# tiems90/mosaic

Hardware: AMD Instinct MI355X
Metric: PIP-join points/sec (H3 res 9) at 1/2/4/8 GPUs + achieved HBM GB/s (higher is better)
Workload: dtype f64

## Files before the change

mosaic_amd/csrc/kernels.hip:

```cpp
#include <hip/hip_runtime.h>
#include <stdint.h>

#include <map>
#include <mutex>

#define H3T_QUAL static __constant__ const
#include "h3_core.h"
#include "bng_core.h"
#include "pip_core.h"
#include "h3_ring.h"
#include "kernels.h"
#include "raster.h"

namespace mgpu {

#ifndef MGPU_BLOCK
#define MGPU_BLOCK 64
#endif
constexpr int kBlock = MGPU_BLOCK;
constexpr int kItems = 4;
constexpr int kTile = kBlock * kItems;
constexpr int kStreamBlock = 256;
static_assert(kTile <= 1024, "point-in-tile indices are 10 bits");

// ... 267 lines not shown
  h3::FastHex f = h3::fast_hex2d(lat, lon, res_o, t.k_res > 0 ? t.k_res : h3::k_of_res(res_o), kAllFaces);
  if (f.tie) {
    if (a.tie_host) {
      if (!SLOW) tie_record(a.tie_queue, a.tie_cap, input_pos(a, p), px, py, h3::lattice_key(f.face, f.ijk));
    } else if (!SLOW) {
      *tie = true;
      return Range{0, 0, 0};
    } else {
      route_point(a, p, px, py, &f, tie);
    }
  }
  return probe_range(t, h3::face_ijk_to_h3_fast(f.face, f.ijk, res_o));
}

__device__ __forceinline__ bool chip_is_core(const ChipTableView& t, const Range& r, uint32_t j) {
  return j < 16 ? ((r.core >> j) & 1) : (t.chip_flags[r.first + j] & kChipCore) != 0;
}

template <bool SLOW, int CAND_CAP, int STASH, bool PT_STASH = false>
__device__ __forceinline__ void phase1_item(const ChipTableView& t, int li, const Range& r, double px, double py,
                                            bool& any_tie, uint32_t* s_ncand, uint16_t* s_cand_pj,
                                            double2* s_cand_xy, uint32_t* s_first, uint16_t* s_cnt,
                                            uint32_t* s_mask, uint32_t answer = kNoCellAns, bool deep = false) {
  if (!SLOW && r.count > (uint32_t)kMaskBits) any_tie = true;
  if (deep && r.count == 1 && (r.core & kCoreWhole)) answer = 1u;
  if (answer != kNoCellAns) {
    s_first[li] = r.first;
    if (SLOW) s_cnt[li] = (uint16_t)r.count;
    s_mask[li] = answer;
    return;
  }
  const uint32_t nj = r.count < (uint32_t)kMaskBits ? r.count : (uint32_t)kMaskBits;
  const uint32_t lowm = nj >= 32 ? 0xFFFFFFFFu : ((1u << nj) - 1);
  uint32_t border = ~r.core & lowm;
  for (uint32_t j = 16; j < nj; j++)
    if (t.chip_flags[r.first + j] & kChipCore) border &= ~(1u << j);
  uint32_t mask = lowm & ~border;
  if (border) {
    if (PT_STASH) s_cand_xy[li] = make_double2(px, py);
    const uint32_t nb = __popc(border);
    uint32_t j0 = atomicAdd(s_ncand, nb);
    for (uint32_t b = border; b; b &= b - 1) {
      const uint32_t j = __builtin_ctz(b);
      if (j0 < (uint32_t)CAND_CAP) {
        s_cand_pj[j0] = (uint16_t)(li | (j << 10));
        if (!PT_STASH && j0 < (uint32_t)STASH) s_cand_xy[j0] = make_double2(px, py);
      } else if (!SLOW) {
        any_tie = true;
      } else if (pip::chip_contains_strips(t, r.first + j, px, py)) {
        mask |= 1u << j;
      }
      j0++;
    }
  }
  s_first[li] = r.first;
  if (SLOW) s_cnt[li] = (uint16_t)(r.count > 0xFFFF ? 0xFFFF : r.count);
  s_mask[li] = mask;
}



#ifdef MGPU_STAMPS
#define MGPU_STAMP(ph)                                                              \
  do {                                                                              \
    if (threadIdx.x == 0) {                                                         \
      const uint64_t now = wall_clock64();                                          \
      if ((ph) > 0) atomicAdd(&a.counters[9 + (ph)], (unsigned long long)(now - st_t)); \
      st_t = now;                                                                   \
    }                                                                               \
  } while (0)
#else
#define MGPU_STAMP(ph) \
  do {             \
  } while (0)
#endif

constexpr int kChunk = 4096;
constexpr int kGTile = kTile;
constexpr int kChunkTiles = kChunk / kGTile;
constexpr int kGCandCap = 3 * kTile;
constexpr int kGMixCap = kTile;


template <int IS, bool SLOW, int G = 0>
__device__ __forceinline__ void join_tile(const JoinArgs& a, const uint32_t tile) {
  __shared__ uint32_t s_ncand, s_nmix;
  __shared__ uint32_t s_wave_tot[kBlock / 64];
  __shared__ uint32_t s_first[kTile];
  __shared__ __attribute__((aligned(16))) uint32_t s_mask[kTile];
  __shared__ uint16_t s_cnt[(SLOW || G == 0) ? kTile : 1];
  constexpr int kCap = G ? kGCandCap : kCandCap, kMix = G ? kGMixCap : kMixCap;
  constexpr int kStash = stash_of<G>();
  __shared__ __attribute__((aligned(16))) uint8_t s_buf[G ? kStash * 16 + kCap * 2 + kMix * 2 : kOutCap * 6];
  double2* s_cand_xy = (double2*)s_buf;
  uint16_t* s_cand_pj = (uint16_t*)(s_buf + kStash * 16);
  uint16_t* s_mix = (uint16_t*)(s_buf + kStash * 16 + kCap * 2);
  int32_t* s_out_poly = (int32_t*)s_buf;
  uint16_t* s_out_li = (uint16_t*)(s_buf + kOutCap * 4);
  __shared__ uint16_t s_gidx[G == 2 ? kTile : 1];

  const uint32_t chunk = G ? tile / kChunkTiles : 0u;
  const int64_t gbase = (int64_t)chunk * kChunk;
  const int64_t lbase = gbase + (int64_t)(tile % kChunkTiles) * kGTile;
  uint32_t gcount = 0;
  if (G) {
    const int64_t left = a.n - gbase;
    const uint32_t nm = G == 2 ? a.chunk_mixed[chunk] : (uint32_t)(left <= 0 ? 0 : (left < kChunk ? left : kChunk));
    const uint32_t t0 = (tile % kChunkTiles) * kGTile;
    if (nm <= t0) return;
    gcount = nm - t0 < (uint32_t)kGTile ? nm - t0 : (uint32_t)kGTile;
    if (G == 2)
      for (uint32_t li = threadIdx.x; li < (uint32_t)kTile; li += kBlock)
        s_gidx[li] = li < gcount ? a.mixed_idx[lbase + li] : (uint16_t)0;
  }
  uint32_t ckp[G == 1 ? 4 : 1];
  if (G == 1 && a.in_chunk_pairs) {
    const uint32_t s0 = 4u * threadIdx.x;
    if (s0 + 3 < gcount) {
      const uint4 q = *(const uint4*)(a.pos_of + lbase + s0);
      ckp[0] = q.x, ckp[1] = q.y, ckp[2] = q.z, ckp[3] = q.w;
    } else {
#pragma unroll
      for (int i = 0; i < 4; i++) ckp[i] = s0 + i < gcount ? a.pos_of[lbase + s0 + i] : 0u;
    }
  }
#define MGPU_PT(li) (G == 2 ? gbase + (int64_t)s_gidx[li] : G == 1 ? lbase + (li) : (int64_t)tile * kTile + (li))
#define MGPU_VALID(li) (G ? (uint32_t)(li) < gcount : (int64_t)tile * kTile + (li) < a.n)


#ifdef MGPU_STAMPS
  uint64_t st_t = 0;
#endif
  if (threadIdx.x == 0) {
    s_ncand = 0;
    s_nmix = 0;
  }
  __syncthreads();
  const ChipTableView& t = a.chips;
  const int64_t base = (int64_t)tile * kTile;
  const bool res_match = a.res_match;

  MGPU_STAMP(0);
  bool any_tie = false, any_bad = false;
  uint32_t n_tie_pts = 0;
#ifndef MGPU_NT_POINTS
#define MGPU_NT_POINTS 1
#endif
#if MGPU_NT_POINTS
#define MGPU_LDPT(ptr) __builtin_nontemporal_load(ptr)
#else
#define MGPU_LDPT(ptr) (*(ptr))
#endif
  if (!G && !SLOW && kBlock == 64 && t.raster_mode != kRasterNone && res_match && (IS == MGPU_H3 || a.res == t.res)) {
    const int lane = threadIdx.x;
    double bx[kItems], by[kItems];
#pragma unroll
    for (int k = 0; k < kItems; k++) {
      const int64_t p = base + k * kBlock + lane;
      bx[k] = by[k] = 0.0;
      if (p < a.n) {
        bx[k] = MGPU_LDPT(&a.x[p]);
        by[k] = MGPU_LDPT(&a.y[p]);
      }
    }
    uint32_t ri[kItems], gix[kItems], sb[kItems];
#pragma unroll
    for (int k = 0; k < kItems; k++) {
// ... 53 lines not shown
      if (q < nlist) {
        bool ok, tie;
        uint32_t gi;
        Range r = chip_probe<IS, SLOW>(a, base + li, px, py, &ok, &tie, &gi);
        if (gi != kNoEntry) r = grid_range(t.grid[gi], t.cell_ans_row != nullptr);
        any_tie |= tie;
        phase1_item<SLOW, kCap, kStash, point_stash<G>()>(t, li, r, px, py, any_tie, &s_ncand, s_cand_pj, s_cand_xy, s_first, s_cnt, s_mask);
      }
    }
  } else if (IS == MGPU_BNG) {
    double bx[kItems], by[kItems];
#pragma unroll
    for (int k = 0; k < kItems; k++) {
      const int li = k * kBlock + threadIdx.x;
      bx[k] = by[k] = 0.0;
      if (MGPU_VALID(li)) {
        const int64_t p = MGPU_PT(li);
        bx[k] = MGPU_LDPT(&a.x[p]);
        by[k] = MGPU_LDPT(&a.y[p]);
      }
    }
    Range r[kItems];
    uint32_t gi[kItems];
#pragma unroll
    for (int k = 0; k < kItems; k++) {
      r[k] = Range{0, 0, 0};
      gi[k] = kNoEntry;
      if (MGPU_VALID(k * kBlock + threadIdx.x) && pt_valid(a.valid, a.valid_off, MGPU_PT(k * kBlock + threadIdx.x))) {
        bool ok, tie;
        r[k] = chip_probe<IS, SLOW>(a, MGPU_PT(k * kBlock + threadIdx.x), bx[k], by[k], &ok, &tie, &gi[k]);
        any_bad |= !ok;
      }
    }
    uint64_t ge[kItems];
#pragma unroll
    for (int k = 0; k < kItems; k++) ge[k] = gi[k] != kNoEntry ? t.grid[gi[k]] : 0;
    uint32_t av[kItems];
#pragma unroll
    for (int k = 0; k < kItems; k++) {
      av[k] = kNoCellAns;
      if (t.cell_ans_row && (ge[k] & kCellAnsFlag)) {
        const uint32_t eI = (uint32_t)bng::d2i(bx[k]), nI = (uint32_t)bng::d2i(by[k]), ed = t.bng_edge;
        const uint32_t col = div_fix(eI, ed, t.bng_inv_edge), row = div_fix(nI, ed, t.bng_inv_edge);
        const uint32_t u = div_fix(eI - col * ed, t.cell_ans_sw, t.cell_ans_inv_sw);
        const uint32_t v = div_fix(nI - row * ed, t.cell_ans_sw, t.cell_ans_inv_sw);
        const uint32_t ai = t.cell_ans_row[row - (uint32_t)t.dense[0].b0] + cell_ans_index(ge[k]);
        const uint16_t m = t.cell_ans[((size_t)ai * t.cell_ans_g + v) * t.cell_ans_g + u];
        if (m != kCellAnsMixed) av[k] = m;
      }
    }
#pragma unroll
    for (int k = 0; k < kItems; k++) {
      if (gi[k] != kNoEntry) r[k] = grid_range(ge[k], t.cell_ans_row != nullptr);
      phase1_item<SLOW, kCap, kStash, point_stash<G>()>(t, k * kBlock + threadIdx.x, r[k], bx[k], by[k], any_tie, &s_ncand, s_cand_pj,
                        s_cand_xy, s_first, s_cnt, s_mask, av[k]);
    }
  } else if (!SLOW && G == 1 && IS == MGPU_H3 && a.bin_key != nullptr) {
    uint32_t kv[kItems];
    double bx[kItems], by[kItems];
#pragma unroll
    for (int k = 0; k < kItems; k++) {
      const int li = k * kBlock + threadIdx.x;
      kv[k] = kKeyNone;
      bx[k] = by[k] = 0.0;
      if (MGPU_VALID(li)) {
        const int64_t p = MGPU_PT(li);
        kv[k] = MGPU_LDPT(&a.bin_key[p]);
        bx[k] = MGPU_LDPT(&a.x[p]);
        by[k] = MGPU_LDPT(&a.y[p]);
      }
    }
    uint64_t ge[kItems];
#pragma unroll
    for (int k = 0; k < kItems; k++) ge[k] = kv[k] < kKeyTie ? t.grid[kv[k] & kKeyIndex] : 0ull;
#pragma unroll
    for (int k = 0; k < kItems; k++) {
      const bool hit = kv[k] < kKeyTie;
      any_bad |= kv[k] == kKeyBad;
      any_tie |= kv[k] == kKeyTie;
      const Range r = hit ? grid_range(ge[k], t.cell_ans_row != nullptr) : Range{0, 0, 0};
      phase1_item<SLOW, kCap, kStash, point_stash<G>()>(t, k * kBlock + threadIdx.x, r, bx[k], by[k], any_tie, &s_ncand,
                                                        s_cand_pj, s_cand_xy, s_first, s_cnt, s_mask, kNoCellAns,
                                                        hit && (kv[k] & kKeyDeep) != 0u);
    }
  } else {
    double nx = 0.0, ny = 0.0;
    if (MGPU_VALID(threadIdx.x)) {
      nx = MGPU_LDPT(&a.x[MGPU_PT(threadIdx.x)]);
      ny = MGPU_LDPT(&a.y[MGPU_PT(threadIdx.x)]);
    }
#pragma unroll 1
    for (int k = 0; k < kItems; k++) {
      const int li = k * kBlock + threadIdx.x;
      const int64_t p = MGPU_PT(li);
      Range r{0, 0, 0};
      const double px = nx, py = ny;
      if (k + 1 < kItems && MGPU_VALID(li + kBlock)) {
        nx = MGPU_LDPT(&a.x[MGPU_PT(li + kBlock)]);
        ny = MGPU_LDPT(&a.y[MGPU_PT(li + kBlock)]);
      }
      bool deep = false;
      if (MGPU_VALID(li) && pt_valid(a.valid, a.valid_off, p)) {
        bool ok, tie;
        uint32_t gi;
        r = chip_probe<IS, SLOW>(a, p, px, py, &ok, &tie, &gi, &deep);
        if (gi != kNoEntry) r = grid_range(t.grid[gi], t.cell_ans_row != nullptr);
        n_tie_pts += (SLOW && tie) ? 1u : 0u;
        any_bad |= !ok;
        any_tie |= tie;
      }
      phase1_item<SLOW, kCap, kStash, point_stash<G>()>(t, li, r, px, py, any_tie, &s_ncand, s_cand_pj, s_cand_xy, s_first, s_cnt, s_mask,
                                                        kNoCellAns, deep);
    }
  }
  count_wave(&a.counters[2], any_bad);
  if (SLOW) {
    const uint32_t wt = wave_sum_u32(n_tie_pts);
    if ((threadIdx.x & 63) == 0 && wt) atomicAdd(&a.counters[1], (unsigned long long)wt);
  }
  if (!SLOW && __syncthreads_or(any_tie)) {
    if (threadIdx.x == 0) {
      const unsigned int q = atomicAdd(a.n_dirty, 1u);
      a.dirty[q] = tile;
      if (!G) {
        a.tile_count[tile] = 0;
        a.tile_where[tile] = kNoDst;
      }
    }
    return;
  }
  __syncthreads();
  MGPU_STAMP(1);
  const uint32_t ncand = s_ncand < (uint32_t)kCap ? s_ncand : (uint32_t)kCap;
  if (threadIdx.x == 0 && s_ncand) atomicAdd(&a.group_cand[G ? chunk : tile / kScanGroup], s_ncand);

  bool redo = false;
  for (uint32_t c = threadIdx.x; c < ncand; c += kBlock) {
    const uint32_t pj = s_cand_pj[c];
    const int li = pj & 1023;
    const uint32_t ch = s_first[li] + (pj >> 10);
    const int64_t p = MGPU_PT(li);
    double px, py;
    if (point_stash<G>() || c < (uint32_t)kStash) {
      const double2 q = s_cand_xy[point_stash<G>() ? (uint32_t)li : c];
      px = q.x;
      py = q.y;
    } else {
      px = a.x[p];
      py = a.y[p];
    }
    const int q = pip::chip_quick(t, ch, px, py, nullptr);
    bool hit = q == pip::kQuickYes;
    if (q >= pip::kQuickStrips) {
      const uint32_t m = atomicAdd(&s_nmix, 1u);
      if (m < (uint32_t)kMix && (SLOW || q == pip::kQuickStrips)) {
        s_mix[m] = (uint16_t)c;
      } else if (!SLOW) {
        redo = true;
      } else {
        hit = q == pip::kQuickStrips ? pip::chip_contains_mixed(t, ch, px, py)
                                     : pip::chip_locate(t, ch, px, py) == pip::kInterior;
      }
    }
    if (hit) atomicOr(&s_mask[li], 1u << (pj >> 10));
  }
  if (!SLOW && __syncthreads_or(redo)) {
// ... 13 lines not shown
#ifdef MGPU_STATS
  uint32_t st_edges = 0;
#endif
  bool walked = false;
#if MGPU_EDGE_PAR
  if (MGPU_EDGE_PAR == 1 || G == 2)
  if (!SLOW && kBlock == 64 && nmix > 0 && nmix <= 64) {
    constexpr uint32_t kBufBytes = sizeof(s_buf);
    constexpr uint32_t kWalkBytes = 64 * (8 + 8 + 4 + 4 + 4 + 4 + 1);
    constexpr uint32_t kFlatCap = kBufBytes > kWalkBytes ? kBufBytes - kWalkBytes : 0;
    const uint32_t lane = threadIdx.x;
    uint32_t pj = 0, ch = 0, eb = 0, ne = 0;
    int li = 0;
    bool one = false;
    uint8_t fl = 0;
    double px = 0.0, py = 0.0;
    if (lane < nmix) {
      const uint32_t c = s_mix[lane];
      pj = s_cand_pj[c];
      li = pj & 1023;
      ch = s_first[li] + (pj >> 10);
      if (point_stash<G>() || c < (uint32_t)kStash) {
        const double2 q = s_cand_xy[point_stash<G>() ? (uint32_t)li : c];
        px = q.x;
        py = q.y;
      } else {
        px = a.x[MGPU_PT(li)];
        py = a.y[MGPU_PT(li)];
      }
      const ChipHdr& H = t.chip_hdr[ch];
      const uint32_t strip = H.strip_base + (uint32_t)strip_of(py, H.env[1], H.inv_h, (int)H.n_strips);
      one = H.single_ring != 0;
      fl = H.flags;
      eb = t.strip_edge[strip];
      ne = t.strip_edge[strip + 1] - eb;
    }
    uint32_t inc = ne;
    for (int d = 1; d < 64; d <<= 1) {
      const uint32_t u = (uint32_t)__shfl_up((int)inc, d);
      if ((int)lane >= d) inc += u;
    }
    const uint32_t total = (uint32_t)__shfl((int)inc, 63), off = inc - ne;
    if (total <= kFlatCap) {
      __syncthreads();
      double* s_wx = (double*)s_buf;
      double* s_wy = s_wx + 64;
      uint32_t* s_web = (uint32_t*)(s_wy + 64);
      uint32_t* s_woff = s_web + 64;
      uint32_t* s_bnd = s_woff + 64;
      uint32_t* s_par = s_bnd + 64;
      uint8_t* s_wone = (uint8_t*)(s_par + 64);
      uint8_t* s_walk = s_wone + 64;
      s_wx[lane] = px;
      s_wy[lane] = py;
      s_web[lane] = eb;
      s_woff[lane] = off;
      s_bnd[lane] = 0;
      s_par[lane] = 0;
      s_wone[lane] = one ? 1 : 0;
      for (uint32_t k = 0; k < ne; k++) s_walk[off + k] = (uint8_t)lane;
      __syncthreads();
      const double4* E4 = (const double4*)t.edges;
#ifndef MGPU_EDGE_PAR_STEPS
#define MGPU_EDGE_PAR_STEPS 4
#endif
      constexpr int kS = MGPU_EDGE_PAR_STEPS;
      const uint32_t e_safe = s_web[s_walk[0]];
      for (uint32_t f0 = 0; f0 < total; f0 += 64 * kS) {
        double4 R[kS];
        uint32_t wm[kS], we[kS];
#pragma unroll
        for (int k = 0; k < kS; k++) {
          const uint32_t f = f0 + lane + 64u * k;
          wm[k] = f < total ? s_walk[f] : 0u;
          we[k] = f < total ? s_web[wm[k]] + (f - s_woff[wm[k]]) : 0u;
          R[k] = E4[f < total ? we[k] : e_safe];
        }
#pragma unroll
        for (int k = 0; k < kS; k++) {
          const uint32_t f = f0 + lane + 64u * k;
          if (f >= total) continue;
          const int bits = pip::count_segment(R[k].x, R[k].y, R[k].z, R[k].w, s_wx[wm[k]], s_wy[wm[k]]);
          if (!bits) continue;
          const uint32_t rb = s_wone[wm[k]] ? 1u : 1u << t.edge_ring[we[k]];
          if (bits & pip::kRingOnSegment) atomicOr(&s_bnd[wm[k]], rb);
          if (bits & 2) atomicXor(&s_par[wm[k]], rb);
        }
      }
      __syncthreads();
      if (lane < nmix && pip::strip_verdict(t, ch, one, fl, s_bnd[lane], s_par[lane], px, py))
        atomicOr(&s_mask[li], 1u << (pj >> 10));
      walked = true;
    }
  }
#endif
  if (!walked) {
#if MGPU_SPLIT_WALK
  if (!SLOW && kBlock == 64 && nmix > 0 && nmix <= 32) {
    const uint32_t lg = nmix <= 16 ? 2u : 1u;
    const uint32_t lane = threadIdx.x, m = lane >> lg, sub = lane & ((1u << lg) - 1u);
    uint32_t bnd = 0, par = 0, pj = 0, ch = 0;
    int li = 0;
    bool one = false;
    uint8_t fl = 0;
    double px = 0.0, py = 0.0;
    if (m < nmix) {
      const uint32_t c = s_mix[m];
      pj = s_cand_pj[c];
      li = pj & 1023;
      ch = s_first[li] + (pj >> 10);
      if (point_stash<G>() || c < (uint32_t)kStash) {
        const double2 q = s_cand_xy[point_stash<G>() ? (uint32_t)li : c];
        px = q.x;
        py = q.y;
      } else {
        px = a.x[MGPU_PT(li)];
        py = a.y[MGPU_PT(li)];
      }
      const ChipHdr& H = t.chip_hdr[ch];
      const uint32_t strip = H.strip_base + (uint32_t)strip_of(py, H.env[1], H.inv_h, (int)H.n_strips);
      one = H.single_ring != 0;
      fl = H.flags;
      pip::strip_bits(t, strip, one, px, py, sub * MGPU_EDGE_STEP, MGPU_EDGE_STEP << lg, &bnd, &par);
    }
    for (uint32_t o = 1; o < (1u << lg); o <<= 1) {
      bnd |= (uint32_t)__shfl_xor((int)bnd, (int)o);
      par ^= (uint32_t)__shfl_xor((int)par, (int)o);
    }
    if (m < nmix && sub == 0 && pip::strip_verdict(t, ch, one, fl, bnd, par, px, py))
      atomicOr(&s_mask[li], 1u << (pj >> 10));
  } else
#endif
  for (uint32_t m = threadIdx.x; m < nmix; m += kBlock) {
    const uint32_t c = s_mix[m];
    const uint32_t pj = s_cand_pj[c];
    const int li = pj & 1023;
    const uint32_t ch = s_first[li] + (pj >> 10);
    const int64_t p = MGPU_PT(li);
    double px, py;
    if (point_stash<G>() || c < (uint32_t)kStash) {
      const double2 q = s_cand_xy[point_stash<G>() ? (uint32_t)li : c];
      px = q.x;
      py = q.y;
    } else {
      px = a.x[p];
      py = a.y[p];
    }
    bool hit;
    if (SLOW && (t.chip_hdr[ch].flags & kChipNoStrips)) {
      hit = pip::chip_locate(t, ch, px, py) == pip::kInterior;
    } else {
#ifdef MGPU_STATS
      uint32_t ne = 0;
      hit = pip::chip_contains_mixed(t, ch, px, py, &ne);
      st_edges += ne;
#else
      hit = pip::chip_contains_mixed(t, ch, px, py);
#endif
    }
    if (hit) atomicOr(&s_mask[li], 1u << (pj >> 10));
  }
  }
#ifdef MGPU_STATS
  if (threadIdx.x == 0) {
    atomicAdd(&a.counters[8], (unsigned long long)s_nmix);
  }
  atomicAdd(&a.counters[9], (unsigned long long)st_edges);
#endif
  __syncthreads();

  MGPU_STAMP(3);
  if (G) {
// ... 423 lines not shown
        const int64_t pj = c0 + (int64_t)(b + j / 2) * 128 + 2 * lane + (j & 1);
        if (pj < a.n && pt_valid(a.valid, a.valid_off, pj)) {
          bool ok = true;
          uint32_t g_ = 0, s_ = 0, b_ = kNoPixel;
          if (IS == MGPU_BNG && bng_grid) {
            const uint32_t m = bng_grid_class(a, pj, X[j], Y[j], &ok, &g_);
            ri[j] = m == kPixMixed ? kRasterFull : m;
          } else {
            ri[j] = raster_index<IS>(t, X[j], Y[j], &ok, &g_, &s_, &b_);
          }
          gix[j] = g_;
          sb[j] = s_;
          bi[j] = use_blk ? b_ : kNoPixel;
          any_bad |= !ok;
        }
      }
      uint32_t cl[kPts];
      uint64_t ge[kPts];
#pragma unroll
      for (int j = 0; j < kPts; j++) {
        if (IS == MGPU_BNG && bng_grid) {
          cl[j] = ri[j] == kRasterFull ? kPixMixed : (ri[j] == kNoPixel ? kPixEmpty : ri[j]);
          ge[j] = gix[j];
        } else {
          cl[j] = ri[j] < kRasterFull ? raster_class_blk(t, s_blk, ri[j], bi[j], sb[j], s_band)
                                      : (ri[j] == kRasterFull ? kPixMixed : kPixEmpty);
          ge[j] = (IS == MGPU_BNG && ri[j] < kRasterFull) ? t.grid[gix[j]] : 0ull;
        }
      }
      Code code[kPts];
      bool mixed[kPts];
#pragma unroll
      for (int j = 0; j < kPts; j++) {
        const int64_t pj = c0 + (int64_t)(b + j / 2) * 128 + 2 * lane + (j & 1);
        bool m = cl[j] == kPixMixed;
        if (IS == MGPU_H3) {
          code[j] = (Code)cl[j];
          if (!m && cl[j] != kPixEmpty) {
            const uint32_t c = cl[j];
            pairs += c < t.raster_pc[0] ? 1u : c < t.raster_pc[1] ? 2u : c < t.raster_pc[2] ? 3u : c < t.raster_pc[3] ? 4u
                     : (uint32_t)__popc((uint32_t)(t.raster_cls[c] >> 32));
          }
        } else {
          const uint32_t first = (uint32_t)ge[j], mm = cl[j];
          if (!m && mm && !(mm < 256u && first < (1u << 24))) m = true;
          code[j] = (Code)(m ? kCodeMixed32 : (mm ? (first << 8) | mm : 0u));
          if (!m) pairs += __popc(mm);
        }
        mixed[j] = m && pj < a.n;
      }
#pragma unroll
      for (int k = 0; k < kPB; k++) {
        const int64_t p = c0 + (int64_t)(b + k) * 128 + 2 * lane;
        if (p + 1 < a.n) {
          if (sizeof(Code) == 2) {
            MGPU_ST_INTER((uint32_t)code[2 * k] | ((uint32_t)code[2 * k + 1] << 16), (uint32_t*)(codes + p));
          } else {
            typedef uint32_t u32x2_t __attribute__((ext_vector_type(2)));
            u32x2_t v;
            v.x = (uint32_t)code[2 * k];
            v.y = (uint32_t)code[2 * k + 1];
            MGPU_ST_INTER(v, (u32x2_t*)(codes + p));
          }
        } else if (p < a.n) {
          MGPU_ST_INTER(code[2 * k], &codes[p]);
        }
        const unsigned long long b0 = __ballot(mixed[2 * k]), b1 = __ballot(mixed[2 * k + 1]);
        const uint32_t r0 = nmixed + (uint32_t)__popcll(b0 & below) + (uint32_t)__popcll(b1 & below);
        const uint16_t li = (uint16_t)((b + k) * 128 + 2 * lane);
        if (mixed[2 * k]) sa.mixed_idx[c0 + r0] = li;
        if (mixed[2 * k + 1]) sa.mixed_idx[c0 + r0 + (mixed[2 * k] ? 1u : 0u)] = (uint16_t)(li + 1);
        nmixed += (uint32_t)(__popcll(b0) + __popcll(b1));
      }
    }
    pairs = wave_sum_u32(pairs);
    if (lane == 0) {
      sa.chunk_pairs[ch] = pairs;
      sa.chunk_mixed[ch] = nmixed;
    }
  }
  count_wave(&a.counters[2], any_bad);
}

template <int IS>
__global__ __launch_bounds__(kBlock) MGPU_JOIN_ATTR void pip_mixed_kernel(JoinArgs a) {
  const uint32_t nm = a.chunk_mixed[blockIdx.x];
  if (threadIdx.x == 0 && nm > (uint32_t)kGTile) {
    const uint32_t more = (nm - 1) / kGTile;
    const uint32_t q = atomicAdd(a.n_extra, more);
    for (uint32_t t = 0; t < more; t++) a.extra[q + t] = blockIdx.x * kChunkTiles + 1 + t;
  }
  join_tile<IS, false, 2>(a, blockIdx.x * kChunkTiles);
}

template <int IS>
__global__ __launch_bounds__(kBlock) void pip_mixed_more_kernel(JoinArgs a) {
  const uint32_t n = *a.n_extra;
  for (uint32_t q = blockIdx.x; q < n; q += gridDim.x) {
    join_tile<IS, false, 2>(a, a.extra[q]);
    __syncthreads();
  }
}

template <int IS, int G>
__global__ __launch_bounds__(kBlock) void pip_mixed_fix_kernel(JoinArgs a) {
  const uint32_t nd = *a.n_dirty;
  for (uint32_t q = blockIdx.x; q < nd; q += gridDim.x) {
    join_tile<IS, true, G>(a, a.dirty[q]);
    __syncthreads();
  }
}

#ifndef MGPU_EMIT_LDSBAR
#define MGPU_EMIT_LDSBAR 1
#endif
__device__ __forceinline__ void lds_barrier() {
#if MGPU_EMIT_LDSBAR
  asm volatile("s_waitcnt lgkmcnt(0)\n\ts_barrier" ::: "memory");
#else
  __syncthreads();
#endif
}

__device__ __forceinline__ uint32_t chunk_excl_scan(uint32_t v, uint32_t* s_w, uint32_t* total) {
  const int lane = threadIdx.x & 63, wave = threadIdx.x >> 6;
  const uint32_t incl = wave_incl_scan(v);
  if (lane == 63) s_w[wave] = incl;
  lds_barrier();
  uint32_t before = 0, all = 0;
#pragma unroll
  for (int w = 0; w < kClsBlock / 64; w++) {
    before += w < wave ? s_w[w] : 0u;
    all += s_w[w];
  }
  *total = all;
  return before + incl - v;
}

constexpr int kEmitWin = 2048;
#ifndef MGPU_EMIT_SWZ
#define MGPU_EMIT_SWZ 1
#endif
__device__ __forceinline__ uint32_t emit_swz(uint32_t q) { return MGPU_EMIT_SWZ ? q ^ ((q >> 6) & 63u) : q; }
#ifndef MGPU_EMIT_NT
#define MGPU_EMIT_NT 1
#endif
#ifndef MGPU_EMIT_NT_OTHER
#define MGPU_EMIT_NT_OTHER 0
#endif
#ifndef MGPU_EMIT_WAVES
#define MGPU_EMIT_WAVES 5
#endif
constexpr int kEmitCls = 2048;
constexpr int kEmitMres = 512;
#ifndef MGPU_EMIT_MR
#define MGPU_EMIT_MR 1
#endif
template <int IS>
__global__ __launch_bounds__(kClsBlock) __attribute__((amdgpu_waves_per_eu(MGPU_EMIT_WAVES))) void split_emit_kernel(SplitArgs sa) {
  using Code = typename CodeOf<IS>::T;
  constexpr int kWords = kClsItems * (int)sizeof(Code) / 4;
  static_assert(kWords % 4 == 0 && kWords >= 4, "whole 16-byte code loads per thread (MGPU_CLS_BLOCK 256 or 512)");
  const JoinArgs& a = sa.j;
  const ChipTableView& t = a.chips;
  __shared__ uint32_t s_w[2][kClsBlock / 64];
  __shared__ uint32_t s_poly[kEmitWin];
  __shared__ uint16_t s_pt[kEmitWin];
  __shared__ int32_t s_cp[IS == MGPU_H3 ? kEmitCls : 1];
  __shared__ uint64_t s_mr[MGPU_EMIT_MR ? kEmitMres : 1];
  __shared__ int32_t s_mp[MGPU_EMIT_MR ? kEmitMres : 1];
  if (sa.redo_affected && blockIdx.x < *sa.redo_first && !sa.redo_affected[blockIdx.x]) return;
  const int64_t c0 = (int64_t)blockIdx.x * kChunk;
  const int64_t p0 = c0 + (int64_t)threadIdx.x * kClsItems;
  const Code kMixed = IS == MGPU_H3 ? (Code)kPixMixed : (Code)kCodeMixed32;
  uint32_t cw[kWords];
  if (p0 + kClsItems <= a.n) {
    const uint4* src = (const uint4*)((const Code*)sa.codes + p0);
#pragma unroll
    for (int i = 0; i < kWords / 4; i++) {
      const uint4 v = src[i];
      cw[4 * i] = v.x, cw[4 * i + 1] = v.y, cw[4 * i + 2] = v.z, cw[4 * i + 3] = v.w;
    }
  } else {
#pragma unroll
    for (int i = 0; i < kWords; i++) cw[i] = 0;
    const Code* cs = (const Code*)sa.codes;
    for (int k = 0; k < kClsItems; k++)
      if (p0 + k < a.n) {
        const uint32_t c = cs[p0 + k];
        if (sizeof(Code) == 2)
          cw[k >> 1] |= c << ((k & 1) * 16);
        else
          cw[k] = c;
      }
  }
  uint32_t ncp = 0;
  if (IS == MGPU_H3) {
    ncp = min(min(t.raster_ncls, t.raster_pc[0]), (uint32_t)kEmitCls);
    for (uint32_t i = threadIdx.x; i < ncp; i += kClsBlock) s_cp[i] = t.raster_cls_poly[i];
  }
  constexpr uint32_t kMr = MGPU_EMIT_MR ? (uint32_t)kEmitMres : 0u;
#if MGPU_EMIT_MR
  {
    const uint32_t nm = sa.chunk_mixed[blockIdx.x], nms = nm < kMr ? nm : kMr;
    for (uint32_t i = threadIdx.x; i < nms; i += kClsBlock) {
      const uint64_t v = a.mixed_res[c0 + i];
      const uint32_t m = (uint32_t)(v >> 32);
      s_mr[i] = v;
      s_mp[i] = __popc(m) == 1 ? t.chip_poly[(uint32_t)v + __builtin_ctz(m)] : 0;
    }
  }
#endif
  auto code = [&](int k) -> Code {
    return sizeof(Code) == 2 ? (Code)(cw[k >> 1] >> ((k & 1) * 16)) : (Code)cw[k];
  };
  auto pure = [&](Code c) -> uint64_t {
    if (IS == MGPU_H3) return t.raster_cls[(uint32_t)c];
    return (uint64_t)((uint32_t)c >> 8) | ((uint64_t)((uint32_t)c & 0xFFu) << 32);
  };
  auto mres = [&](uint32_t r) -> uint64_t { return r < kMr ? s_mr[r] : a.mixed_res[c0 + r]; };
  uint32_t nmix = 0;
#pragma unroll
  for (int k = 0; k < kClsItems; k++) nmix += code(k) == kMixed;
  uint32_t all_mixed;
  const uint32_t rank0 = chunk_excl_scan(nmix, s_w[0], &all_mixed);
  uint32_t npair = 0, r = rank0;
#pragma unroll
  for (int k = 0; k < kClsItems; k++) {
    const Code c = code(k);
    if (c == kMixed)
      npair += __popc((uint32_t)(mres(r++) >> 32));
    else if (c != 0) {
      if (IS == MGPU_H3)
        npair += c < t.raster_pc[0]   ? 1u
                 : c < t.raster_pc[1] ? 2u
                 : c < t.raster_pc[2] ? 3u
                 : c < t.raster_pc[3] ? 4u
                                      : (uint32_t)__popc((uint32_t)(pure(c) >> 32));
      else
        npair += (uint32_t)__popc((uint32_t)c & 0xFFu);
    }
  }
  uint32_t total;
  const uint32_t off0 = chunk_excl_scan(npair, s_w[1], &total);
  const uint64_t base = sa.chunk_off[blockIdx.x];
  for (uint32_t w0 = 0; w0 < total; w0 += kEmitWin) {
    if (off0 < w0 + kEmitWin && off0 + npair > w0) {
      uint32_t q = off0;
      r = rank0;
#pragma unroll
      for (int k = 0; k < kClsItems; k++) {
        const Code c = code(k);
        uint64_t v = 0;
        bool has_one = false;
        int32_t one = 0;
        if (c == kMixed) {
          const uint32_t rr = r++;
          if (rr < kMr && __popc((uint32_t)(s_mr[rr] >> 32)) == 1)
            has_one = true, one = s_mp[rr];
          else
            v = mres(rr);
        } else if (IS == MGPU_H3 && c != 0 && (uint32_t)c < ncp)
          has_one = true, one = s_cp[(uint32_t)c];
        else if (c != 0)
          v = pure(c);
        if (has_one) {
          if (q >= w0 && q < w0 + kEmitWin) {
            s_poly[emit_swz(q - w0)] = (uint32_t)one;
            s_pt[emit_swz(q - w0)] = (uint16_t)(threadIdx.x * kClsItems + k);
          }
          q++;
        }
        const uint32_t first = (uint32_t)v;
        for (uint32_t m = (uint32_t)(v >> 32); m; m &= m - 1, q++)
          if (q >= w0 && q < w0 + kEmitWin) {
            s_poly[emit_swz(q - w0)] = (uint32_t)t.chip_poly[first + __builtin_ctz(m)];
            s_pt[emit_swz(q - w0)] = (uint16_t)(threadIdx.x * kClsItems + k);
          }
      }
    }
    lds_barrier();
    const uint32_t cnt = total - w0 < (uint32_t)kEmitWin ? total - w0 : (uint32_t)kEmitWin;
    for (uint32_t i = threadIdx.x; i < cnt; i += kClsBlock) {
      const uint64_t q = base + w0 + i;
      if ((int64_t)q >= sa.capacity) break;
      const int64_t p = c0 + s_pt[emit_swz(i)];
#if MGPU_EMIT_NT
      __builtin_nontemporal_store(sa.point_id ? sa.point_id[p] : sa.id_base + p, &sa.out_point[q]);
      __builtin_nontemporal_store((int32_t)s_poly[emit_swz(i)], &sa.out_poly[q]);
#else
      sa.out_point[q] = sa.point_id ? sa.point_id[p] : sa.id_base + p;
      sa.out_poly[q] = (int32_t)s_poly[emit_swz(i)];
#endif
    }
    lds_barrier();
  }
}

constexpr int kScanBlock = 1024;
constexpr int kScanLds = 24576;
__global__ __launch_bounds__(kScanBlock) void tile_scan_kernel(const uint32_t* __restrict__ gsum,
                                                               const uint32_t* __restrict__ gcand, int64_t ng,
                                                               uint64_t* __restrict__ goff,
                                                               unsigned long long* __restrict__ counters,
                                                               const uint32_t* only_if = nullptr) {
  if (only_if && *only_if == 0) return;
  __shared__ unsigned long long s_w[kScanBlock / 64];
  __shared__ uint32_t s_v[kScanLds];
  __shared__ unsigned long long s_base[kScanBlock];
  const int lane = threadIdx.x & 63, wave = threadIdx.x >> 6;
  const int64_t per = (ng + kScanBlock - 1) / kScanBlock;
  const int64_t b = threadIdx.x * per, e = b + per < ng ? b + per : ng;
  unsigned long long cand = 0, sum = 0;
  const bool lds = ng <= kScanLds;
  if (lds) {
    for (int64_t i = threadIdx.x; i < ng; i += kScanBlock) {
      cand += gcand[i];
      s_v[i] = gsum[i];
    }
    __syncthreads();
    for (int64_t i = b; i < e; i++) sum += s_v[i];
  } else {
    for (int64_t i = b; i < e; i++) {
      cand += gcand[i];
      sum += gsum[i];
    }
  }
  cand = wave_sum_u64(cand);
  if (lane == 0 && cand) atomicAdd(&counters[3], cand);
  unsigned long long incl = sum;
#pragma unroll
  for (int d = 1; d < 64; d <<= 1) {
    const unsigned long long u = __shfl_up(incl, d, 64);
    if (lane >= d) incl += u;
  }
  if (lane == 63) s_w[wave] = incl;
  __syncthreads();
  unsigned long long run = incl - sum, tot = 0;
  for (int w = 0; w < kScanBlock / 64; w++) {
    if (w < wave) run += s_w[w];
    tot += s_w[w];
  }
  if (lds) {
    s_base[threadIdx.x] = run;
// ... 700 lines not shown
__device__ __forceinline__ void bin_gather_lds(const BinArgs& b, int64_t c0, uint32_t m, int nb,
                                               const uint32_t* s_off, const uint32_t* s_loc, uint64_t* s_v) {
  uint32_t pp[kBgItems];
  uint64_t rv[kBgItems];
#pragma unroll
  for (int q = 0; q < kBgItems; q++) {
    const uint32_t lp = q * kBinBlock + threadIdx.x;
    pp[q] = 0xFFFFFFFFu;
    if (lp < m) {
      const uint32_t bi = bin_at(s_loc, nb, lp);
      const uint32_t sl = s_off[bi] + (lp - s_loc[bi]);
      pp[q] = b.perm[sl];
      rv[q] = b.s.j.mixed_res[sl];
    }
  }
#pragma unroll
  for (int q = 0; q < kBgItems; q++)
    if (pp[q] != 0xFFFFFFFFu) s_v[pp[q] - (uint32_t)c0] = rv[q];
}

__global__ __launch_bounds__(kBinBlock) void bin_gather_kernel(BinArgs b) {
  __shared__ uint64_t s_v[kBinChunk];
  __shared__ uint32_t s_off[kBinMax];
  __shared__ uint32_t s_loc[kBinMax];
  __shared__ uint32_t s_w[kBinBlock / 64];
  const int nb = b.nbx * b.nby;
  const int64_t k = blockIdx.x;
  const int64_t n = b.s.j.n, c0 = k * kBinChunk;
  bin_runs(b, k, s_off, s_loc, s_w);
  const int64_t left = n - c0;
  const uint32_t m = left < kBinChunk ? (uint32_t)left : (uint32_t)kBinChunk;
#ifndef MGPU_GATHER_UNROLL
#define MGPU_GATHER_UNROLL 1
#endif
  if (MGPU_GATHER_UNROLL) {
    bin_gather_lds(b, c0, m, nb, s_off, s_loc, s_v);
  } else {
    for (uint32_t lp = threadIdx.x; lp < m; lp += kBinBlock) {
      const uint32_t bi = bin_at(s_loc, nb, lp);
      const uint32_t sl = s_off[bi] + (lp - s_loc[bi]);
      s_v[b.perm[sl] - (uint32_t)c0] = b.s.j.mixed_res[sl];
    }
  }
  __syncthreads();
  constexpr int kPerWave = kChunk / (kBinBlock / 64) * (kBinChunk / kChunk);
  const int lane = threadIdx.x & 63, wave = threadIdx.x >> 6;
  uint32_t np = 0;
  for (int i = wave * kPerWave + lane; i < (wave + 1) * kPerWave; i += 64)
    if ((uint32_t)i < m) {
      const uint64_t v = s_v[i];
      MGPU_ST_INTER(v, &b.res[c0 + i]);
      np += __popc((uint32_t)(v >> 32));
    }
  np = wave_sum_u32(np);
  __syncthreads();
  if (lane == 0) s_w[wave] = np;
  __syncthreads();
  constexpr int kE = kBinChunk / kChunk, kWpe = (kBinBlock / 64) / kE;
  if ((int)threadIdx.x < kE) {
    const int64_t e = k * kE + threadIdx.x;
    if (e * kChunk < n) {
      uint32_t t = 0;
      for (int w = 0; w < kWpe; w++) t += s_w[threadIdx.x * kWpe + w];
      b.s.chunk_pairs[e] = t;
    }
  }
}

__device__ __forceinline__ void bin_answers(const BinArgs& b, int64_t p0, uint64_t* v) {
  const int64_t n = b.s.j.n;
  if (p0 + kBinEmitItems <= n) {
    const ulonglong2* src = (const ulonglong2*)(b.res + p0);
#pragma unroll
    for (int i = 0; i < kBinEmitItems / 2; i++) {
      const ulonglong2 q = src[i];
      v[2 * i] = q.x, v[2 * i + 1] = q.y;
    }
  } else {
#pragma unroll
    for (int k = 0; k < kBinEmitItems; k++) v[k] = p0 + k < n ? b.res[p0 + k] : 0ull;
  }
}

__global__ __launch_bounds__(kClsBlock) __attribute__((amdgpu_waves_per_eu(MGPU_EMIT_WAVES))) void bin_emit_kernel(BinArgs b) {
  const SplitArgs& sa = b.s;
  const ChipTableView& t = sa.j.chips;
  __shared__ uint32_t s_w[kClsBlock / 64];
  __shared__ uint32_t s_poly[kEmitWin];
  __shared__ uint16_t s_pt[kEmitWin];
  const int64_t c0 = (int64_t)blockIdx.x * kChunk;
  const int l0 = threadIdx.x * kBinEmitItems;
  uint64_t v[kBinEmitItems];
  bin_answers(b, c0 + l0, v);
  uint32_t npair = 0;
#pragma unroll
  for (int k = 0; k < kBinEmitItems; k++) npair += __popc((uint32_t)(v[k] >> 32));
  uint32_t total;
  const uint32_t off0 = chunk_excl_scan(npair, s_w, &total);
  const uint64_t base = sa.chunk_off[blockIdx.x];
  for (uint32_t w0 = 0; w0 < total; w0 += kEmitWin) {
    if (off0 < w0 + kEmitWin && off0 + npair > w0) {
      uint32_t q = off0;
#pragma unroll
      for (int k = 0; k < kBinEmitItems; k++) {
        const uint32_t first = (uint32_t)v[k], msk = (uint32_t)(v[k] >> 32);
        if (msk == 1u) {
          if (q >= w0 && q < w0 + kEmitWin) {
            s_poly[emit_swz(q - w0)] = first;
            s_pt[emit_swz(q - w0)] = (uint16_t)(l0 + k);
          }
          q++;
          continue;
        }
        for (uint32_t m = msk; m; m &= m - 1, q++)
          if (q >= w0 && q < w0 + kEmitWin) {
            s_poly[emit_swz(q - w0)] = (uint32_t)t.chip_poly[first + __builtin_ctz(m)];
            s_pt[emit_swz(q - w0)] = (uint16_t)(l0 + k);
          }
      }
    }
    __syncthreads();
    const uint32_t cnt = total - w0 < (uint32_t)kEmitWin ? total - w0 : (uint32_t)kEmitWin;
    for (uint32_t i = threadIdx.x; i < cnt; i += kClsBlock) {
      const uint64_t q = base + w0 + i;
      if ((int64_t)q >= sa.capacity) break;
      const int64_t p = c0 + s_pt[emit_swz(i)];
#if MGPU_EMIT_NT_OTHER
      __builtin_nontemporal_store(sa.point_id ? sa.point_id[p] : sa.id_base + p, &sa.out_point[q]);
      __builtin_nontemporal_store((int32_t)s_poly[emit_swz(i)], &sa.out_poly[q]);
#else
      sa.out_point[q] = sa.point_id ? sa.point_id[p] : sa.id_base + p;
      sa.out_poly[q] = (int32_t)s_poly[emit_swz(i)];
#endif
    }
    __syncthreads();
  }
}

#ifndef MGPU_BIN_JOIN_COUNTS
#define MGPU_BIN_JOIN_COUNTS 1
#endif
static_assert(kBinChunk == kChunk, "one emit chunk per bin chunk");
__global__ __launch_bounds__(kBinBlock) void bin_emit_gather_kernel(BinArgs b) {
  const SplitArgs& sa = b.s;
  const ChipTableView& t = sa.j.chips;
  __shared__ uint64_t s_v[kBinChunk];
  __shared__ uint32_t s_off[kBinMax];
  __shared__ uint32_t s_loc[kBinMax];
  __shared__ uint32_t s_w[kBinBlock / 64];
  __shared__ uint32_t s_poly[kEmitWin];
  __shared__ uint16_t s_pt[kEmitWin];
  const int nb = b.nbx * b.nby;
  const int64_t k = blockIdx.x, n = sa.j.n, c0 = k * kBinChunk;
  bin_runs(b, k, s_off, s_loc, s_w);
  const int64_t left = n - c0;
  const uint32_t m = left < kBinChunk ? (uint32_t)left : (uint32_t)kBinChunk;
  bin_gather_lds(b, c0, m, nb, s_off, s_loc, s_v);
  __syncthreads();
  const int l0 = threadIdx.x * kBgItems;
  uint64_t v[kBgItems];
  uint32_t npair = 0;
#pragma unroll
  for (int q = 0; q < kBgItems; q++) {
    v[q] = (uint32_t)(l0 + q) < m ? s_v[l0 + q] : 0ull;
    npair += __popc((uint32_t)(v[q] >> 32));
  }
  const int lane = threadIdx.x & 63, wave = threadIdx.x >> 6;
// ... 137 lines not shown
    hipLaunchKernelGGL(pair_emit_kernel, dim3((unsigned)((a.n_tiles + kEmitTiles - 1) / kEmitTiles)),
                       dim3(kEmitBlock), 0, s, e, a.n_tiles);
  return hipGetLastError();
}

__global__ __launch_bounds__(256) void tile_unpair_kernel(JoinArgs a, RedoArgs R, int64_t n) {
  const int64_t i = (int64_t)blockIdx.x * 256 + threadIdx.x;
  if (i >= n) return;
  const uint32_t tile = R.list[i];
  const uint32_t c = a.tile_count[tile];
  R.old[i] = c;
  if (c) atomicSub(&a.group_sum[tile / kScanGroup], c);
  a.tile_count[tile] = 0;
  a.tile_where[tile] = kNoDst;
  R.affected[tile] = 1;
  a.dirty[i] = tile;
}

__global__ __launch_bounds__(256) void chunk_unpair_kernel(JoinArgs a, RedoArgs R) {
  __shared__ uint32_t s_w[4];
  const uint32_t chunk = R.list[blockIdx.x];
  const uint32_t nm = a.chunk_mixed[chunk];
  uint32_t mine = 0;
  for (uint32_t i = threadIdx.x; i < nm; i += 256) mine += __popc((uint32_t)(a.mixed_res[(int64_t)chunk * kChunk + i] >> 32));
  mine = wave_sum_u32(mine);
  if ((threadIdx.x & 63) == 0) s_w[threadIdx.x >> 6] = mine;
  __syncthreads();
  if (threadIdx.x == 0) {
    const uint32_t tot = s_w[0] + s_w[1] + s_w[2] + s_w[3];
    R.old[blockIdx.x] = a.group_sum[chunk];
    a.group_sum[chunk] -= tot;
    a.group_cand[chunk] = 0;
    R.affected[chunk] = 1;
    const uint32_t nt = (nm + kGTile - 1) / kGTile;
    const uint32_t q = atomicAdd(a.n_dirty, nt);
    for (uint32_t t = 0; t < nt; t++) a.dirty[q + t] = chunk * kChunkTiles + t;
  }
}

__global__ __launch_bounds__(256) void redo_compare_kernel(const uint32_t* counts, RedoArgs R, int64_t n) {
  const int64_t i = (int64_t)blockIdx.x * 256 + threadIdx.x;
  if (i < n && counts[R.list[i]] != R.old[i]) {
    atomicOr(R.changed, 1u);
    atomicMin(R.first, R.list[i]);
  }
}

hipError_t launch_join_redo(int is, const JoinArgs& a, const EmitArgs& e, const RedoArgs& R, int64_t n, hipStream_t s,
                            bool emit) {
  if (n <= 0) return hipSuccess;
  const unsigned g = (unsigned)((n + 255) / 256);
  hipLaunchKernelGGL(tile_unpair_kernel, dim3(g), dim3(256), 0, s, a, R, n);
  const unsigned fix_blocks = (unsigned)(n < kFixGrid ? n : kFixGrid);
  if (is == MGPU_H3)
    hipLaunchKernelGGL(pip_fix_kernel<MGPU_H3>, dim3(fix_blocks), dim3(kBlock), 0, s, a);
  else
    hipLaunchKernelGGL(pip_fix_kernel<MGPU_BNG>, dim3(fix_blocks), dim3(kBlock), 0, s, a);
  hipLaunchKernelGGL(redo_compare_kernel, dim3(g), dim3(256), 0, s, (const uint32_t*)a.tile_count, R, n);
  hipLaunchKernelGGL(tile_scan_kernel, dim3(1), dim3(kScanBlock), 0, s, a.group_sum, a.group_cand,
                     (a.n_tiles + kScanGroup - 1) / kScanGroup, e.group_off, a.counters, (const uint32_t*)R.changed);
  EmitArgs er = e;
  er.redo_first = R.first;
  er.redo_affected = R.affected;
  if (emit)
    hipLaunchKernelGGL(pair_emit_kernel, dim3((unsigned)((a.n_tiles + kEmitTiles - 1) / kEmitTiles)),
                       dim3(kEmitBlock), 0, s, er, a.n_tiles);
  return hipGetLastError();
}

int64_t split_chunk() { return kChunk; }
int64_t split_chunk_tiles() { return kChunkTiles; }
int64_t split_chunks(int64_t n) { return (n + kChunk - 1) / kChunk; }

static int resident_blocks(const void* kernel, int block, size_t lds) {
  int dev = 0, cus = 0, per = 0;
  hipGetDevice(&dev);
  hipDeviceGetAttribute(&cus, hipDeviceAttributeMultiprocessorCount, dev);
  if (hipOccupancyMaxActiveBlocksPerMultiprocessor(&per, kernel, block, lds) != hipSuccess || per < 1) per = 1;
  return std::max(cus, 1) * per;
}

template <int IS>
static void launch_emit(const SplitArgs& a, int64_t nc, hipStream_t s) {
  hipLaunchKernelGGL(split_emit_kernel<IS>, dim3((unsigned)nc), dim3(kClsBlock), 0, s, a);
}

template <int IS>
static void launch_split_t(const SplitArgs& a, hipStream_t s, hipEvent_t after_classify, hipEvent_t after_mixed, bool emit) {
  const int64_t nc = split_chunks(a.j.n);
  const ChipTableView& ct = a.j.chips;
  const size_t nblk = (IS == MGPU_H3 && ct.raster_blk) ? (size_t)ct.raster_bnx * ct.raster_bny : 0;
  const size_t lds = IS == MGPU_H3 ? ((nblk + 1) & ~(size_t)1) * 2 + (size_t)ct.raster_nband * 4 : 0;
  const int64_t wg = (nc + kCfyBlock / 64 - 1) / (kCfyBlock / 64);
  if (lds > 64 * 1024) {
    hipFuncSetAttribute((const void*)classify_pair_kernel<IS>, hipFuncAttributeMaxDynamicSharedMemorySize, (int)lds);
    hipFuncSetAttribute((const void*)classify_wave_kernel<IS>, hipFuncAttributeMaxDynamicSharedMemorySize, (int)lds);
  }
  if (MGPU_CFY_PAIR && ((((uintptr_t)a.j.x) | ((uintptr_t)a.j.y)) & 15) == 0) {
    const int64_t grid = std::min<int64_t>(wg, (int64_t)resident_blocks((const void*)classify_pair_kernel<IS>, kCfyBlock, lds));
    hipLaunchKernelGGL(classify_pair_kernel<IS>, dim3((unsigned)grid), dim3(kCfyBlock), lds, s, a, nc);
  } else {
    const int64_t grid = std::min<int64_t>(wg, (int64_t)resident_blocks((const void*)classify_wave_kernel<IS>, kCfyBlock, lds));
    hipLaunchKernelGGL(classify_wave_kernel<IS>, dim3((unsigned)grid), dim3(kCfyBlock), lds, s, a, nc);
  }
  if (after_classify) hipEventRecord(after_classify, s);
  hipLaunchKernelGGL(pip_mixed_kernel<IS>, dim3((unsigned)nc), dim3(kBlock), 0, s, a.j);
  const int64_t more = std::min<int64_t>(nc, (int64_t)resident_blocks((const void*)pip_mixed_more_kernel<IS>, kBlock, 0));
  hipLaunchKernelGGL(pip_mixed_more_kernel<IS>, dim3((unsigned)more), dim3(kBlock), 0, s, a.j);
  const int64_t fix = nc * kChunkTiles < kFixGrid ? nc * kChunkTiles : kFixGrid;
  hipLaunchKernelGGL((pip_mixed_fix_kernel<IS, 2>), dim3((unsigned)fix), dim3(kBlock), 0, s, a.j);
  if (after_mixed) hipEventRecord(after_mixed, s);
  hipLaunchKernelGGL(tile_scan_kernel, dim3(1), dim3(kScanBlock), 0, s, a.chunk_pairs, a.j.group_cand, nc,
                     a.chunk_off, a.j.counters);
  if (emit) launch_emit<IS>(a, nc, s);
}

hipError_t launch_split(int is, const SplitArgs& a, hipStream_t s, hipEvent_t after_classify, hipEvent_t after_mixed,
                        bool emit) {
  if (a.j.n <= 0) return hipSuccess;
  if (is == MGPU_H3)
    launch_split_t<MGPU_H3>(a, s, after_classify, after_mixed, emit);
  else
    launch_split_t<MGPU_BNG>(a, s, after_classify, after_mixed, emit);
  return hipGetLastError();
}

hipError_t launch_split_redo(int is, const SplitArgs& sa, const RedoArgs& R, int64_t n, hipStream_t s, bool emit) {
  if (n <= 0) return hipSuccess;
  const int64_t nc = split_chunks(sa.j.n);
  hipLaunchKernelGGL(chunk_unpair_kernel, dim3((unsigned)n), dim3(256), 0, s, sa.j, R);
  const int64_t most = n * kChunkTiles;
  const unsigned fix = (unsigned)(most < kFixGrid ? most : kFixGrid);
  if (is == MGPU_H3)
    hipLaunchKernelGGL((pip_mixed_fix_kernel<MGPU_H3, 2>), dim3(fix), dim3(kBlock), 0, s, sa.j);
  else
    hipLaunchKernelGGL((pip_mixed_fix_kernel<MGPU_BNG, 2>), dim3(fix), dim3(kBlock), 0, s, sa.j);
  hipLaunchKernelGGL(redo_compare_kernel, dim3((unsigned)((n + 255) / 256)), dim3(256), 0, s,
                     (const uint32_t*)sa.chunk_pairs, R, n);
  hipLaunchKernelGGL(tile_scan_kernel, dim3(1), dim3(kScanBlock), 0, s, sa.chunk_pairs, sa.j.group_cand, nc,
                     sa.chunk_off, sa.j.counters, (const uint32_t*)R.changed);
  SplitArgs sr = sa;
  sr.redo_first = R.first;
  sr.redo_affected = R.affected;
  if (!emit) return hipGetLastError();
  if (is == MGPU_H3)
    launch_emit<MGPU_H3>(sr, nc, s);
  else
    launch_emit<MGPU_BNG>(sr, nc, s);
  return hipGetLastError();
}

hipError_t launch_split_emit(int is, const SplitArgs& a, hipStream_t s) {
  if (a.j.n <= 0) return hipSuccess;
  const int64_t nc = split_chunks(a.j.n);
  if (is == MGPU_H3)
    launch_emit<MGPU_H3>(a, nc, s);
  else
    launch_emit<MGPU_BNG>(a, nc, s);
  return hipGetLastError();
}

int64_t bin_chunk() { return kBinChunk; }
int64_t bin_chunks(int64_t n) { return (n + kBinChunk - 1) / kBinChunk; }
int64_t bin_groups(int64_t n) { return (bin_chunks(n) + kBinGroup - 1) / kBinGroup; }
int32_t bin_max() { return kBinMax; }

static void launch_bin_output(const BinArgs& a, hipStream_t s, bool emit) {
// ... 78 lines not shown
```

Before: 98.22 billion.

## Add lean mixed-tile join path and shrink emit kernel LDS footprint

Adds a LEAN variant of join_tile, used by default in pip_mixed_kernel. It loads all point coordinates up front, probes chips directly, and recomputes walk-state values from LDS after the edge loop instead of keeping them live in registers. The split emit kernel also changes. Its class-poly table becomes dynamic LDS sized to the number of classes actually staged, and the single-poly mixed results are packed into s_mr so the separate s_mp array is dropped. Its waves-per-EU hint rises for H3 while BNG and bin-emit keep the old value. Together these aim to cut register and LDS pressure so occupancy goes up, at the cost of extra LDS reads and a host-side read of table fields to size the launch.

Measured after the change: 103.8 billion (median of 6 runs). +5.6%, better.

```diff
diff --git a/mosaic_amd/csrc/kernels.hip b/mosaic_amd/csrc/kernels.hip
--- a/mosaic_amd/csrc/kernels.hip
+++ b/mosaic_amd/csrc/kernels.hip
@@ -373,7 +373,7 @@
 constexpr int kGMixCap = kTile;
 
 
-template <int IS, bool SLOW, int G = 0>
+template <int IS, bool SLOW, int G = 0, bool LEAN = false>
 __device__ __forceinline__ void join_tile(const JoinArgs& a, const uint32_t tile) {
   __shared__ uint32_t s_ncand, s_nmix;
   __shared__ uint32_t s_wave_tot[kBlock / 64];
@@ -593,6 +593,33 @@
       phase1_item<SLOW, kCap, kStash, point_stash<G>()>(t, k * kBlock + threadIdx.x, r, bx[k], by[k], any_tie, &s_ncand,
                                                         s_cand_pj, s_cand_xy, s_first, s_cnt, s_mask, kNoCellAns,
                                                         hit && (kv[k] & kKeyDeep) != 0u);
+    }
+  } else if (LEAN) {
+    double bx[kItems], by[kItems];
+#pragma unroll
+    for (int k = 0; k < kItems; k++) {
+      const int li = k * kBlock + threadIdx.x;
+      bx[k] = by[k] = 0.0;
+      if (MGPU_VALID(li)) {
+        bx[k] = MGPU_LDPT(&a.x[MGPU_PT(li)]);
+        by[k] = MGPU_LDPT(&a.y[MGPU_PT(li)]);
+      }
+    }
+#pragma unroll
+    for (int k = 0; k < kItems; k++) {
+      const int li = k * kBlock + threadIdx.x;
+      Range r{0, 0, 0};
+      bool deep = false;
+      if (MGPU_VALID(li) && pt_valid(a.valid, a.valid_off, MGPU_PT(li))) {
+        bool ok, tie;
+        uint32_t gi;
+        r = chip_probe<IS, SLOW>(a, MGPU_PT(li), bx[k], by[k], &ok, &tie, &gi, &deep);
+        if (gi != kNoEntry) r = grid_range(t.grid[gi], t.cell_ans_row != nullptr);
+        any_bad |= !ok;
+        any_tie |= tie;
+      }
+      phase1_item<SLOW, kCap, kStash, point_stash<G>()>(t, li, r, bx[k], by[k], any_tie, &s_ncand, s_cand_pj, s_cand_xy, s_first, s_cnt,
+                                                        s_mask, kNoCellAns, deep);
     }
   } else {
     double nx = 0.0, ny = 0.0;
@@ -772,12 +799,20 @@
           if (f >= total) continue;
           const int bits = pip::count_segment(R[k].x, R[k].y, R[k].z, R[k].w, s_wx[wm[k]], s_wy[wm[k]]);
           if (!bits) continue;
-          const uint32_t rb = s_wone[wm[k]] ? 1u : 1u << t.edge_ring[we[k]];
+          const uint32_t rb = s_wone[wm[k]] ? 1u : 1u << t.edge_ring[LEAN ? s_web[wm[k]] + (f - s_woff[wm[k]]) : we[k]];
           if (bits & pip::kRingOnSegment) atomicOr(&s_bnd[wm[k]], rb);
           if (bits & 2) atomicXor(&s_par[wm[k]], rb);
         }
       }
       __syncthreads();
+      if (LEAN) {
+        asm volatile("" : "+v"(pj));
+        one = s_wone[lane] != 0;
+        px = s_wx[lane];
+        py = s_wy[lane];
+        li = pj & 1023;
+        ch = s_first[li] + (pj >> 10);
+      }
       if (lane < nmix && pip::strip_verdict(t, ch, one, fl, s_bnd[lane], s_par[lane], px, py))
         atomicOr(&s_mask[li], 1u << (pj >> 10));
       walked = true;
@@ -1367,6 +1402,9 @@
   count_wave(&a.counters[2], any_bad);
 }
 
+#ifndef MGPU_MIXED_LEAN
+#define MGPU_MIXED_LEAN 1
+#endif
 template <int IS>
 __global__ __launch_bounds__(kBlock) MGPU_JOIN_ATTR void pip_mixed_kernel(JoinArgs a) {
   const uint32_t nm = a.chunk_mixed[blockIdx.x];
@@ -1375,7 +1413,7 @@
     const uint32_t q = atomicAdd(a.n_extra, more);
     for (uint32_t t = 0; t < more; t++) a.extra[q + t] = blockIdx.x * kChunkTiles + 1 + t;
   }
-  join_tile<IS, false, 2>(a, blockIdx.x * kChunkTiles);
+  join_tile<IS, false, 2, MGPU_MIXED_LEAN != 0>(a, blockIdx.x * kChunkTiles);
 }
 
 template <int IS>
@@ -1434,15 +1472,30 @@
 #define MGPU_EMIT_NT_OTHER 0
 #endif
 #ifndef MGPU_EMIT_WAVES
-#define MGPU_EMIT_WAVES 5
+#define MGPU_EMIT_WAVES 7
+#endif
+#ifndef MGPU_EMIT_WAVES_BNG
+#define MGPU_EMIT_WAVES_BNG 5
+#endif
+#ifndef MGPU_BIN_EMIT_WAVES
+#define MGPU_BIN_EMIT_WAVES 5
 #endif
 constexpr int kEmitCls = 2048;
 constexpr int kEmitMres = 512;
 #ifndef MGPU_EMIT_MR
 #define MGPU_EMIT_MR 1
 #endif
+__host__ __device__ inline uint32_t emit_cls_staged(const ChipTableView& t) {
+  const uint32_t n = t.raster_ncls < t.raster_pc[0] ? t.raster_ncls : t.raster_pc[0];
+  return n < (uint32_t)kEmitCls ? n : (uint32_t)kEmitCls;
+}
+template <int N>
+__device__ __forceinline__ void emit_forget(uint32_t (&w)[N]) {
+#pragma unroll
+  for (int i = 0; i < N; i++) asm volatile("" : "+v"(w[i]));
+}
 template <int IS>
-__global__ __launch_bounds__(kClsBlock) __attribute__((amdgpu_waves_per_eu(MGPU_EMIT_WAVES))) void split_emit_kernel(SplitArgs sa) {
+__global__ __launch_bounds__(kClsBlock) __attribute__((amdgpu_waves_per_eu(IS == MGPU_H3 ? MGPU_EMIT_WAVES : MGPU_EMIT_WAVES_BNG))) void split_emit_kernel(SplitArgs sa) {
   using Code = typename CodeOf<IS>::T;
   constexpr int kWords = kClsItems * (int)sizeof(Code) / 4;
   static_assert(kWords % 4 == 0 && kWords >= 4, "whole 16-byte code loads per thread (MGPU_CLS_BLOCK 256 or 512)");
@@ -1451,9 +1504,8 @@
   __shared__ uint32_t s_w[2][kClsBlock / 64];
   __shared__ uint32_t s_poly[kEmitWin];
   __shared__ uint16_t s_pt[kEmitWin];
-  __shared__ int32_t s_cp[IS == MGPU_H3 ? kEmitCls : 1];
   __shared__ uint64_t s_mr[MGPU_EMIT_MR ? kEmitMres : 1];
-  __shared__ int32_t s_mp[MGPU_EMIT_MR ? kEmitMres : 1];
+  extern __shared__ int32_t s_cp[];
   if (sa.redo_affected && blockIdx.x < *sa.redo_first && !sa.redo_affected[blockIdx.x]) return;
   const int64_t c0 = (int64_t)blockIdx.x * kChunk;
   const int64_t p0 = c0 + (int64_t)threadIdx.x * kClsItems;
@@ -1481,7 +1533,7 @@
   }
   uint32_t ncp = 0;
   if (IS == MGPU_H3) {
-    ncp = min(min(t.raster_ncls, t.raster_pc[0]), (uint32_t)kEmitCls);
+    ncp = emit_cls_staged(t);
     for (uint32_t i = threadIdx.x; i < ncp; i += kClsBlock) s_cp[i] = t.raster_cls_poly[i];
   }
   constexpr uint32_t kMr = MGPU_EMIT_MR ? (uint32_t)kEmitMres : 0u;
@@ -1491,8 +1543,7 @@
     for (uint32_t i = threadIdx.x; i < nms; i += kClsBlock) {
       const uint64_t v = a.mixed_res[c0 + i];
       const uint32_t m = (uint32_t)(v >> 32);
-      s_mr[i] = v;
-      s_mp[i] = __popc(m) == 1 ? t.chip_poly[(uint32_t)v + __builtin_ctz(m)] : 0;
+      s_mr[i] = __popc(m) == 1 ? (uint64_t)(uint32_t)t.chip_poly[(uint32_t)v + __builtin_ctz(m)] | (1ull << 32) : v;
     }
   }
 #endif
@@ -1510,6 +1561,7 @@
   uint32_t all_mixed;
   const uint32_t rank0 = chunk_excl_scan(nmix, s_w[0], &all_mixed);
   uint32_t npair = 0, r = rank0;
+  emit_forget(cw);
 #pragma unroll
   for (int k = 0; k < kClsItems; k++) {
     const Code c = code(k);
@@ -1533,6 +1585,7 @@
     if (off0 < w0 + kEmitWin && off0 + npair > w0) {
       uint32_t q = off0;
       r = rank0;
+      emit_forget(cw);
 #pragma unroll
       for (int k = 0; k < kClsItems; k++) {
         const Code c = code(k);
@@ -1541,10 +1594,9 @@
         int32_t one = 0;
         if (c == kMixed) {
           const uint32_t rr = r++;
-          if (rr < kMr && __popc((uint32_t)(s_mr[rr] >> 32)) == 1)
-            has_one = true, one = s_mp[rr];
-          else
-            v = mres(rr);
+          v = mres(rr);
+          if (rr < kMr && __popc((uint32_t)(v >> 32)) == 1)
+            has_one = true, one = (int32_t)(uint32_t)v, v = 0;
         } else if (IS == MGPU_H3 && c != 0 && (uint32_t)c < ncp)
           has_one = true, one = s_cp[(uint32_t)c];
         else if (c != 0)
@@ -2411,7 +2463,7 @@
   }
 }
 
-__global__ __launch_bounds__(kClsBlock) __attribute__((amdgpu_waves_per_eu(MGPU_EMIT_WAVES))) void bin_emit_kernel(BinArgs b) {
+__global__ __launch_bounds__(kClsBlock) __attribute__((amdgpu_waves_per_eu(MGPU_BIN_EMIT_WAVES))) void bin_emit_kernel(BinArgs b) {
   const SplitArgs& sa = b.s;
   const ChipTableView& t = sa.j.chips;
   __shared__ uint32_t s_w[kClsBlock / 64];
@@ -2715,7 +2767,8 @@
 
 template <int IS>
 static void launch_emit(const SplitArgs& a, int64_t nc, hipStream_t s) {
-  hipLaunchKernelGGL(split_emit_kernel<IS>, dim3((unsigned)nc), dim3(kClsBlock), 0, s, a);
+  const size_t lds = IS == MGPU_H3 ? (size_t)emit_cls_staged(a.j.chips) * 4 : 0;
+  hipLaunchKernelGGL(split_emit_kernel<IS>, dim3((unsigned)nc), dim3(kClsBlock), lds, s, a);
 }
 
 template <int IS>
```
